# Wangshihu12/Voxel-SLAM

Measured on AMD Instinct MI355X. Metric: local-BA iterations/sec (200k pts, W=10), higher is better.
Workload: dtype f64

## Files before the change

include/voxelba.h:

```cpp
#ifndef VOXELBA_H
#define VOXELBA_H

#include <stddef.h>
#include <stdint.h>

#ifdef __cplusplus
extern "C" {
#endif

#define VBA_CLUSTER_LEN 10
#define VBA_POSE_LEN 12
#define VBA_STATE_LEN 25
#define VBA_IMU_PRE_LEN 304
#define VBA_DIM 15
#define VBA_MAX_WIN 16

enum vba_status {
  VBA_OK = 0,
  VBA_ERR_NO_DEVICE = 1,
  VBA_ERR_BAD_ARG = 2,
  VBA_ERR_UNSUPPORTED_WINDOW = 3,
  VBA_ERR_TOO_FEW_VOXELS = 4,
  VBA_ERR_OPT_STATE = 5,
  VBA_ERR_HIP = 6,
// ... 124 lines not shown

int vba_pgo_optimize(vba_ctx *ctx, int n, double *poses, int m, const double *edges, int n_prior, const double *priors,
                     int n_updates, double relin_threshold, double *stats);

typedef int (*vba_allreduce_fn)(void *user, void *buf_dev, size_t n_doubles, void *stream);
int vba_set_allreduce(vba_ctx *ctx, vba_allreduce_fn fn, void *user);
int vba_rccl_get_unique_id(void *out128);
int vba_rccl_init(vba_ctx *ctx, const void *unique_id128, int rank, int n_ranks);
int vba_set_rccl_comm(vba_ctx *ctx, void *nccl_comm);
int vba_shard_owner(int64_t kx, int64_t ky, int64_t kz, int n_ranks);
int vba_set_shard(vba_ctx *ctx, int rank, int n_ranks);

int vba_timing_enable(vba_ctx *ctx, int on);
int vba_timing_calibration_read(vba_ctx *ctx, size_t n_bytes);
int vba_timing_select(vba_ctx *ctx, const char *name);
int vba_timing_sample_every(vba_ctx *ctx, int n);
int vba_timing_null_span(vba_ctx *ctx);
int vba_timing_reset(vba_ctx *ctx);
int vba_timing_get(vba_ctx *ctx, const char *name, double *total_us, int *count);

int vba_lm_begin(vba_ctx *ctx, const double *poses, int thd_num);
int vba_lm_refresh_eigen(vba_ctx *ctx);
int vba_timing_launch_hessian(vba_ctx *ctx);
int vba_lm_iterate(vba_ctx *ctx, int *accepted, int *stop);
int vba_lm_end(vba_ctx *ctx, double *poses, double *hess, double *resis2);
#define VBA_SOLVE_LIDAR 0
#define VBA_SOLVE_LI 1
#define VBA_SOLVE_DENSE 2
#define VBA_SOLVE_E_PACKED 1
#define VBA_SOLVE_COPY_RAW 2
#define VBA_SOLVE_FROM_RAW 4
#define VBA_SOLVE_GRAVITY 8
#define VBA_SOLVE_DENSE_MASK 16
int vba_debug_solve(vba_ctx *ctx, int kind, int W, int flags, const double *H, const double *g, double u, double v, double *dx, double *q1);

int vba_io_save_pcd(const char *path, int n, const double *xyz);
int vba_io_load_pcd(const char *path, int cap, double *xyz, double *intensity , int *n_out);
int vba_io_save_pose(const char *path, int n, const double *states, const double *v6);
int vba_io_read_lidarstate(const char *path, int cap, double *states, double *v6 , int *n_out);

#define VBA_BTC_ROW_LEN 19

typedef struct vba_btc_config {
  int skip_near_num;
  int candidate_num;
  float rough_dis_threshold;
  float similarity_threshold;
  float icp_threshold;
  float normal_threshold;
  float dis_threshold;
  int occupy_len;
} vba_btc_config;

typedef struct vba_btc_db vba_btc_db;

typedef struct vba_btc_result {
  int loop_id;
  double score;
  double t[3];
  double R[9];
} vba_btc_result;

typedef struct vba_btc_candidate {
  int frame;
  int votes;
  int match_len;
// ... 82 lines not shown
```

voxel-slam_amd/capi.py:

```python
from __future__ import annotations

import ctypes as C
import os
import subprocess

import numpy as np

_PKG = os.path.dirname(os.path.abspath(__file__))
LIB_PATH = os.environ.get("VBA_LIB") or os.path.join(_PKG, "libvoxelba.so")
_dp = C.POINTER(C.c_double)

OK = 0
ERR_NO_DEVICE, ERR_BAD_ARG, ERR_UNSUPPORTED_WINDOW, ERR_TOO_FEW_VOXELS, ERR_OPT_STATE, ERR_HIP, ERR_CAPACITY, ERR_IO, ERR_UNSUPPORTED, ERR_SINGULAR = range(1, 11)

EXPORTS = [
    "vba_default_options", "vba_create", "vba_destroy", "vba_status_string", "vba_last_error", "vba_synchronize",
    "vba_factor_clear", "vba_factor_push_voxels", "vba_factor_size", "vba_factor_acc_evaluate2",
    "vba_factor_evaluate_only_residual", "vba_factor_read_back", "vba_factor_occupied_slots", "vba_factor_occupancy_masks",
    "vba_lidar_ba_damping_iter", "vba_li_ba_damping_iter", "vba_last_lm_trace",
    "vba_imu_preintegrate", "vba_imu_give_evaluate",
    "vba_map_cut_voxel", "vba_map_pvec_update_cut_voxel", "vba_scan_var_init", "vba_scan_down_sampling_voxel", "vba_scan_down_sampling_pvec", "vba_scan_down_sampling_close", "vba_scan_undistort", "vba_odom_lio_state_estimation_kdtree", "vba_odom_kdtree_reset", "vba_odom_kdtree_size", "vba_odom_kdtree_points", "vba_gba_build", "vba_hba_add_edge", "vba_hba_global", "vba_map_cut_voxel_fix", "vba_map_recut", "vba_map_margi", "vba_map_slide", "vba_map_prune", "vba_map_reset",
    "vba_map_num_roots", "vba_map_num_slide_roots", "vba_map_stats", "vba_map_dump_leaves", "vba_map_dump_plane_var", "vba_odom_lio_state_estimation",
    "vba_set_allreduce", "vba_rccl_get_unique_id", "vba_rccl_init", "vba_set_rccl_comm", "vba_shard_owner", "vba_set_shard",
    "vba_timing_enable", "vba_timing_calibration_read", "vba_timing_select", "vba_timing_sample_every", "vba_timing_launch_hessian", "vba_timing_null_span", "vba_timing_reset", "vba_timing_get",
# ... 587 lines not shown

    def factor_occupancy(self) -> float:
        n = C.c_longlong(0)
        self._chk(self.lib.vba_factor_occupied_slots(self.h, C.byref(n)))
        return n.value / max(self.size(), 1)

    def factor_occupancy_masks(self):
        m = np.zeros(self.size(), dtype=np.uint32)
        self._chk(self.lib.vba_factor_occupancy_masks(self.h, m.ctypes.data_as(C.POINTER(C.c_uint))))
        return m

    def last_trace(self):
        rows = np.zeros((64, 5))
        n = self.lib.vba_last_lm_trace(self.h, _p(rows), C.c_int(64))
        return rows[:n].copy()

    def lidar_ba_damping_iter(self, poses, max_iter=3, thd_num=2):
        poses = _c(poses).copy(); n = 6 * self.W
        H = np.empty((n, n)); resis = np.zeros(2); conv = C.c_int(0)
        st = self.lib.vba_lidar_ba_damping_iter(self.h, _p(poses), _p(H), _p(resis), C.c_int(max_iter), C.c_int(thd_num), C.byref(conv))
        if st == ERR_TOO_FEW_VOXELS:
            return dict(poses=poses, hess=H, resis=resis, converge=False, status=-1, trace=self.last_trace())
        self._chk(st)
        return dict(poses=poses, hess=H, resis=resis, converge=bool(conv.value), status=0, trace=self.last_trace())

    def li_ba_damping_iter(self, states, imus, gravity=False, max_iter=3):
        states = _c(states).copy(); imus = _c(imus).copy()
        n = 15 * self.W + (3 if gravity else 0)
        H = np.empty((n, n)); resis = np.zeros(2)
        self._chk(self.lib.vba_li_ba_damping_iter(self.h, _p(states), _p(imus), C.c_int(int(gravity)), C.c_int(max_iter), _p(H), _p(resis)))
        return dict(states=states, imus=imus, hess=H, resis=resis, trace=self.last_trace())

    SOLVE_KINDS = {"lidar": 0, "li": 1, "dense": 2}
    SOLVE_FLAGS = {"e_packed": 1, "copy_raw": 2, "from_raw": 4, "gravity": 8, "dense_mask": 16}

    def debug_solve(self, kind, W, H, g, u, v=2.0, **flags):
        f = 0
        for k, on in flags.items():
            f |= self.SOLVE_FLAGS[k] if on else 0
        H = _c(H); g = _c(g); n = len(g)
        nc = 1 if kind == "dense" else (self.opt.lm_spec if 0 < self.opt.lm_spec < 4 else 4)
        dx = np.zeros((nc, n)); q1 = np.zeros(nc)
        self._chk(self.lib.vba_debug_solve(self.h, C.c_int(self.SOLVE_KINDS[kind]), C.c_int(W), C.c_int(f), _p(H), _p(g),
                                           C.c_double(u), C.c_double(v), _p(dx), _p(q1)))
        return dx, q1

    def lm_begin(self, poses, thd_num=2):
        poses = _c(poses)
        self._chk(self.lib.vba_lm_begin(self.h, _p(poses), C.c_int(thd_num)))

    def lm_iterate(self, sync=True):
        if not sync:
            self._chk(self.lib.vba_lm_iterate(self.h, None, None))
            return None
        acc = C.c_int(0); stop = C.c_int(0)
        self._chk(self.lib.vba_lm_iterate(self.h, C.byref(acc), C.byref(stop)))
        return bool(acc.value), bool(stop.value)

    def lm_refresh_eigen(self):
        self._chk(self.lib.vba_lm_refresh_eigen(self.h))

    def lm_end(self, fetch=True):
        if not fetch:
            self._chk(self.lib.vba_lm_end(self.h, None, None, None))
            return None
        n = 6 * self.W
        poses = np.empty((self.W, 12)); H = np.empty((n, n)); resis = np.zeros(2)
# ... 329 lines not shown
```

voxel-slam_amd/csrc/vba_kernels_factor.hpp:

```cpp
#pragma once
#include <hip/hip_runtime.h>
#include "vba_eig3.hpp"

namespace vba {

struct FactorView {
  double *cl;
  double *fix;
  double *coe;
  double *eigval;
  double *eigvec;
  double *pcr;
  unsigned int *occ;
  int *tiles;
  int vs;
  int W;
};

__host__ __device__ inline int mask_bucket(unsigned int m, int nb) {
  constexpr int C[11][11] = {{1, 0, 0, 0, 0, 0, 0, 0, 0, 0, 0}, {1, 1, 0, 0, 0, 0, 0, 0, 0, 0, 0}, {1, 2, 1, 0, 0, 0, 0, 0, 0, 0, 0}, {1, 3, 3, 1, 0, 0, 0, 0, 0, 0, 0},
                             {1, 4, 6, 4, 1, 0, 0, 0, 0, 0, 0}, {1, 5, 10, 10, 5, 1, 0, 0, 0, 0, 0}, {1, 6, 15, 20, 15, 6, 1, 0, 0, 0, 0},
                             {1, 7, 21, 35, 35, 21, 7, 1, 0, 0, 0}, {1, 8, 28, 56, 70, 56, 28, 8, 1, 0, 0}, {1, 9, 36, 84, 126, 126, 84, 36, 9, 1, 0},
                             {1, 10, 45, 120, 210, 252, 210, 120, 45, 10, 1}};
  int p = 0;
// ... 163 lines not shown
__device__ __forceinline__ double wave_sum(double x) {
  for (int m = 32; m >= 1; m >>= 1) x += __shfl_xor(x, m, 64);
  return x;
}

__device__ __forceinline__ double dpp_mov_f64(double x, double old, const int ctrl, const int row_mask) {
  const long long xi = __double_as_longlong(x), oi = __double_as_longlong(old);
  int lo = (int)xi, hi = (int)(xi >> 32);
  const int olo = (int)oi, ohi = (int)(oi >> 32);
  switch (ctrl) {
    case 0xB1: lo = __builtin_amdgcn_update_dpp(olo, lo, 0xB1, 0xF, 0xF, false); hi = __builtin_amdgcn_update_dpp(ohi, hi, 0xB1, 0xF, 0xF, false); break;
    case 0x4E: lo = __builtin_amdgcn_update_dpp(olo, lo, 0x4E, 0xF, 0xF, false); hi = __builtin_amdgcn_update_dpp(ohi, hi, 0x4E, 0xF, 0xF, false); break;
    case 0x141: lo = __builtin_amdgcn_update_dpp(olo, lo, 0x141, 0xF, 0xF, false); hi = __builtin_amdgcn_update_dpp(ohi, hi, 0x141, 0xF, 0xF, false); break;
    case 0x140: lo = __builtin_amdgcn_update_dpp(olo, lo, 0x140, 0xF, 0xF, false); hi = __builtin_amdgcn_update_dpp(ohi, hi, 0x140, 0xF, 0xF, false); break;
    case 0x142: lo = __builtin_amdgcn_update_dpp(olo, lo, 0x142, 0xA, 0xF, false); hi = __builtin_amdgcn_update_dpp(ohi, hi, 0x142, 0xA, 0xF, false); break;
    default: lo = __builtin_amdgcn_update_dpp(olo, lo, 0x143, 0xC, 0xF, false); hi = __builtin_amdgcn_update_dpp(ohi, hi, 0x143, 0xC, 0xF, false); break;
  }
  (void)row_mask;
  return __longlong_as_double(((long long)hi << 32) | (unsigned int)lo);
}
__device__ __forceinline__ double group8_sum(double x) {
  x += dpp_mov_f64(x, x, 0xB1, 0xF);
  x += dpp_mov_f64(x, x, 0x4E, 0xF);
  x += dpp_mov_f64(x, x, 0x141, 0xF);
  return x;
}
__device__ __forceinline__ double wave_sum_to_lane63(double x) {
  x += dpp_mov_f64(x, x, 0xB1, 0xF);
  x += dpp_mov_f64(x, x, 0x4E, 0xF);
  x += dpp_mov_f64(x, x, 0x141, 0xF);
  x += dpp_mov_f64(x, x, 0x140, 0xF);
  x += dpp_mov_f64(x, 0.0, 0x142, 0xA);
  x += dpp_mov_f64(x, 0.0, 0x143, 0xC);
  return x;
}

struct LmDev;
template <int W>
struct LmInit {
  double x[12 * W];
  LmDev *dst;
  int on, dbg;
};
template <int W>
__device__ __forceinline__ void lm_init_store(const LmInit<W> &a, int tid, int nt);

template <int W, int TV>
struct ResCfg {
  static constexpr int NT = ((TV * W + 63) / 64) * 64;
  static constexpr int NF = NT / TV;
  static constexpr int KPT = (10 + NF - 1) / NF;
  static_assert(TV <= 64 && (TV & (TV - 1)) == 0 && NT % TV == 0, "the voxel threads are the first TV lanes of wave 0");
  static_assert(W * 12 <= NT, "one thread per pose scalar");
};

template <int W, int TV, bool STAMPS>
__global__ __launch_bounds__((ResCfg<W, TV>::NT)) void k_residual_s(FactorView f, const double *__restrict__ poses, int head, int end,
                                                                  double *__restrict__ partial, const int *__restrict__ gate,
                                                                  long long *__restrict__ stamps, LmInit<W> init) {
  using C = ResCfg<W, TV>;
  __shared__ double T[10][W][TV];
  __shared__ double S[10][TV];
  __shared__ double sp[W * 12];
  const int gate_v = gate ? *gate : 1;
  const int tid = threadIdx.x, vl = tid % TV, fi = tid / TV;
  const int v = head + blockIdx.x * TV + vl;
// ... 576 lines not shown
```

voxel-slam_amd/csrc/vba_kernels_li.hpp:

```cpp
#pragma once
#include <hip/hip_runtime.h>
#include "vba_hostmath.hpp"
#include "vba_li_order.hpp"

namespace vba {

constexpr int LI_MAX_W = 16;
constexpr int LI_MAX_N = 15 * LI_MAX_W + 3;

struct LiDev {
  int W, n, nb, gravity, gauge, F;
  double imu_coef;
  double ex[LI_MAX_W * 12];
  double ext[LI_MAX_W * 12];
  double tstamp[LI_MAX_W];
  double rimu[2];
  double ext_spec[LM_SPEC][LI_MAX_W * 12];
  double ginc_spec[LM_SPEC][4];
  double binc_spec[LM_SPEC][LI_MAX_W * 6];
};

__device__ __forceinline__ void li_state(const double *pose12, const double *ex12, double t, vbh::State &s) {
  s.t = t;
#pragma unroll
// ... 168 lines not shown
  using LC = LdltCfg<NP>;
  extern __shared__ __attribute__((aligned(16))) double lds[];
  const int sb = blockIdx.x;
  constexpr size_t LSCR = (size_t)LC::LTOT > (size_t)NMAX * (NMAX + 1) / 2 ? (size_t)LC::LTOT : (size_t)NMAX * (NMAX + 1) / 2;
  double *Lst = GL ? lscratch + (size_t)sb * LSCR : lds, *Tp = GL ? lds : Lst + LC::LTOT, *P = Tp + NP * LC::LS;
  double *hd = P + NP * 8, *gs = hd + NMAX, *dsh = gs + NMAX, *xs = dsh + NMAX, *dxs = xs + NP, *red8 = dxs + NMAX;
  int *ord = (int *)(red8 + 32);
  const int tid = threadIdx.x;
  const long long t_begin = clock64();
  constexpr int NLB = (2 * W - 1) * 225, NLOW = NLB + 45 * W + 9, QH = (NLOW + NT - 1) / NT, NL = 36 * W * W, QL = (NL + NT - 1) / NT;
  const int nlow = NLB + (grav ? 45 * W + 9 : 0);
  double hv[QH], lv[QL];
#pragma unroll
  for (int q = 0; q < QH; q++) {
    const int e = tid + NT * q, ec = e < nlow ? e : 0;
    int idx;
    if (ec < NLB) { const int blk = ec / 225, a = (blk + 1) >> 1, b = a - (blk & 1); idx = li_hb_pair(a, b) + (ec - 225 * blk); }
    else idx = li_hb_ne1(W) + 45 * W + (ec - NLB);
    hv[q] = himu[idx];
  }
  if (!copy_raw) {
#pragma unroll
    for (int q = 0; q < QL; q++) {
      const int e = tid + NT * q, ec = e < NL ? e : NL - 1;
      const int row = ec / (6 * W), col = ec - row * (6 * W);
      lv[q] = tl_fetch<W>(red, row, col);
    }
  }
  double gimu_v = 0.0, glid_v = 0.0;
  if (tid < n) {
    gimu_v = gimu[tid];
    if (!copy_raw && tid < 15 * W) { const int a = tid / 15, lr = tid - 15 * a; glid_v = (lr < 6) ? red[C2::GB + 6 * a + lr] : 0.0; }
  }
  const int stop = s->stop, calc = s->is_calc_hess, iter0 = s->iter, dbg = sb == 0 ? s->pad : 0, use_spec = s->use_spec;
  const double u0 = s->u, v0 = s->v, rimu0 = li->rimu[0], rlid0 = copy_raw ? 0.0 : red[C2::RB];
  if (stop || use_spec) return;
  double u = u0;
  { double vb = v0; for (int k = 0; k < sb; k++) { u = u * vb; vb = 2 * vb; } }
  if ((dbg & 16) && tid == 0) s->stamps[0] = t_begin;
  const double *__restrict__ src = (copy_raw && !calc) ? raw : red;
  if (copy_raw) {
    if (calc && sb == 0)
      for (int t = tid; t < C2::NOUT2; t += NT) raw[t] = src[t];
#pragma unroll
    for (int q = 0; q < QL; q++) {
      const int e = tid + NT * q, ec = e < NL ? e : NL - 1;
      const int row = ec / (6 * W), col = ec - row * (6 * W);
      lv[q] = tl_fetch<W>(src, row, col);
    }
    if (tid < 15 * W) { const int a = tid / 15, lr = tid - 15 * a; glid_v = (lr < 6) ? src[C2::GB + 6 * a + lr] : 0.0; }
  }
  if (tid == 0 && calc && sb == 0) {
    const double rl = copy_raw ? src[C2::RB] : rlid0, r = coef * 0.5 * rimu0 + rl;
    s->r1 = r; if (iter0 == 0) s->resis_first = r;
    if ((dbg & 32) && iter0 < 3) { s->stamps[58 + 2 * iter0] = __double_as_longlong(rimu0); s->stamps[59 + 2 * iter0] = __double_as_longlong(rl); }
  }
  double *stage = Lst;
  for (int e = tid; e < n * (n + 1) / 2; e += NT) stage[e] = 0.0;
  __syncthreads();
#pragma unroll
  for (int q = 0; q < QH; q++) {
    const int e = tid + NT * q;
    if (e < nlow) {
      int R, Cc;
      if (e < NLB) { const int blk = e / 225, rc = e - 225 * blk, a = (blk + 1) >> 1, b = a - (blk & 1); R = 15 * a + rc / 15; Cc = 15 * b + rc % 15; }
      else if (e < NLB + 45 * W) { const int q2 = e - NLB, k = q2 / (15 * W); R = 15 * W + k; Cc = q2 - k * 15 * W; }
      else { const int q2 = e - NLB - 45 * W; R = 15 * W + q2 / 3; Cc = 15 * W + q2 % 3; }
// ... 9 lines not shown
    if (e < NL && col <= row) {
      const int R = 15 * (row / 6) + row % 6, Cc = 15 * (col / 6) + col % 6;
      stage[R * (R + 1) / 2 + Cc] += lv[q];
    }
  }
  __syncthreads();
  if ((dbg & 16) && tid == 0) s->stamps[51] = clock64();
  if (tid < n) {
    double h = 1.0, g = 0.0;
    if (tid >= gauge) {
      h = stage[tid * (tid + 1) / 2 + tid];
      g = coef * gimu_v + glid_v;
    }
    hd[tid] = h; gs[tid] = g; dsh[tid] = fabs(h + u * h);
  }
  __syncthreads();
  if ((dbg & 16) && tid == 0) s->stamps[52] = clock64();
  if (tid < n) ord[tid] = li_ord(tid, W);
  __syncthreads();
  auto elem = [&](int i, int j) -> double {
    const int jc = j < n ? j : n - 1, ic = i < n ? i : n - 1;
    const int pj = ord[jc], pi = ord[ic];
    const int rr = pi > pj ? pi : pj, cc = pi > pj ? pj : pi;
    double a = stage[rr * (rr + 1) / 2 + cc];
    a = (rr < gauge || cc < gauge) ? ((rr == cc) ? 1.0 : 0.0) : a;
    a = (i == j) ? a + u * a : a;
    a = (i == n) ? -gs[pj] : a;
    a = (i > n || i < j) ? 0.0 : a;
    return (j >= n) ? ((i == j) ? 1.0 : 0.0) : a;
  };
  long long *stamps = ((dbg & 16) != 0) ? s->stamps : nullptr;
  if (stamps && tid == 0) stamps[1] = clock64();
  auto live = [&](int kb) -> unsigned { return li_live(kb, W, n, NP); };
  if constexpr (DENSE_MASK) ldlt_mfma<NP, NT>(Lst, Tp, P, n, elem, stamps, LdltDense());
  else ldlt_mfma<NP, NT>(Lst, Tp, P, n, elem, stamps, live);
  if (stamps && tid == 0) stamps[3] = clock64();
  if (tid < n) xs[tid] = Lst[LC::lat(n, tid)];
  __syncthreads();
  const double x = ldlt_backsub<NP>(Lst, xs, n);
  if (stamps && tid == 0) stamps[4] = clock64();
  if (tid < n) dxs[ord[tid]] = x;
  __syncthreads();
  double *gl = red8 + 16;
  if (grav && tid < 3) {
    if (sb == 0) { const double gn = li->ext[9 + tid] + dxs[n - 3 + tid]; gl[tid] = gn; }
    else li->ginc_spec[sb][tid] = dxs[n - 3 + tid];
  }
  __syncthreads();
  if (tid < W) {
    double E[9];
    so3_exp_dev(dxs + 15 * tid, E);
    const double *R = s->x + 12 * tid;
    double *Rt = (sb == 0 ? s->xt : s->xt_spec[sb]) + 12 * tid;
    double *et = (sb == 0 ? li->ext : li->ext_spec[sb]) + 12 * tid;
    for (int r = 0; r < 3; r++)
      for (int c = 0; c < 3; c++) Rt[3 * r + c] = R[3 * r] * E[c] + R[3 * r + 1] * E[3 + c] + R[3 * r + 2] * E[6 + c];
    for (int k = 0; k < 3; k++) Rt[9 + k] = R[9 + k] + dxs[15 * tid + 3 + k];
    for (int k = 0; k < 9; k++) et[k] = li->ex[12 * tid + k] + dxs[15 * tid + 6 + k];
    if (grav && sb == 0) for (int k = 0; k < 3; k++) et[9 + k] = gl[k];
  }
  if (tid >= 64 && tid < 64 + li->F) {
    const int f = tid - 64;
    if (sb == 0) {
      double *m = imu + 304 * (size_t)f;
      for (int k = 0; k < 3; k++) {
        m[73 + k] = m[67 + k]; m[76 + k] = m[70 + k];
        m[67 + k] += dxs[15 * f + 9 + k]; m[70 + k] += dxs[15 * f + 12 + k];
      }
    } else {
// ... 123 lines not shown
```

voxel-slam_amd/csrc/vba_kernels_lm.hpp:

```cpp
#pragma once
#include <hip/hip_runtime.h>
#include "vba_ldlt.hpp"

namespace vba {

constexpr int LM_SPEC = 4;

struct LmDev {
  double x[VBA_MAX_WIN_DEV * 12];
  double xt[VBA_MAX_WIN_DEV * 12];
  double u, v, r1, r2, q1, resis_first;
  int is_calc_hess, stop, iter, n_trace, all_accepted, last_accepted, max_trace, run_hess, run_res, pad;
  double trace[5 * 64];
  long long stamps[64];
  int spec_n, spec_i, use_spec, pad2;
  double q1_spec[LM_SPEC];
  double xt_spec[LM_SPEC][VBA_MAX_WIN_DEV * 12];
};

template <int W>
__device__ __forceinline__ void lm_init_store(const LmInit<W> &a, int tid, int nt) {
  constexpr int NW = sizeof(LmDev) / 8, XT = offsetof(LmDev, xt) / 8, U = offsetof(LmDev, u) / 8, V = offsetof(LmDev, v) / 8,
                I = offsetof(LmDev, is_calc_hess) / 8;
  static_assert(sizeof(LmDev) % 8 == 0 && offsetof(LmDev, x) == 0 && offsetof(LmDev, u) == 2 * offsetof(LmDev, xt) && 12 * W <= XT, "x and xt lead the image");
// ... 87 lines not shown
      }
  };
  if constexpr (!COPY_RAW) { load_diag(red); load_bulk(red); }
  const double r_v = COPY_RAW ? 0.0 : red[C2::RB];
  double xr[12];
  if (wv == 3 && lane < W)
#pragma unroll
    for (int k = 0; k < 12; k++) xr[k] = s->x[12 * lane + k];
  const long long t_begin = clock64();
  if (stop || use_spec) return;
  double u = u0;
  { double vb = v0; for (int k = 0; k < sb; k++) { u = u * vb; vb = 2 * vb; } }
  if constexpr (COPY_RAW) {
    const double *__restrict__ src = calc ? red : raw;
    if (calc && sb == 0)
      for (int t = tid; t < C2::NOUT2; t += NT) raw[t] = src[t];
    load_diag(src); load_bulk(src);
  }
  double hk[NH], dk[NH];
  int rk[NH];
#pragma unroll
  for (int h = 0; h < NH; h++) {
    const int k = lane + 64 * h;
    hk[h] = k < 6 ? 1.0 : dgt[h] + dge[h];
    dk[h] = fabs(hk[h] + u * hk[h]);
    rk[h] = 0;
  }
#pragma unroll
  for (int j = 0; j < n; j++) {
    const double o = readlane_f64(dk[j >> 6], j & 63);
#pragma unroll
    for (int h = 0; h < NH; h++) rk[h] += (o > dk[h] || (o == dk[h] && j < lane + 64 * h)) ? 1 : 0;
  }
  int prow[T16], pcol[T16];
#pragma unroll
  for (int t = 0; t < T16; t++) {
    const int r = 16 * t + ru, c = 16 * t + cu;
    prow[t] = __shfl(rk[(16 * t) >> 6], (r < n ? r : n - 1) & 63);
    pcol[t] = __shfl(rk[(16 * t) >> 6], (c < n ? c : n - 1) & 63);
  }
  {
    int uu = 0;
#pragma unroll
    for (int ta = 0; ta < T16; ta++)
#pragma unroll
      for (int tb = ta; tb < T16; tb++, uu++) {
        const int row = 16 * ta + ru, col = 16 * tb + cu;
        if (row <= col && col < n) {
          double a = eon[uu] ? tv[uu] + ev[uu] : tv[uu];
          a = (row < 6) ? ((row == col) ? 1.0 : 0.0) : a;
          a = (row == col) ? a + u * a : a;
          const int pr = prow[ta], pc = pcol[tb], hi = pr > pc ? pr : pc, lo = pr > pc ? pc : pr;
          img[hi * (hi + 1) / 2 + lo] = a;
        }
      }
  }
  if (wv == 0)
#pragma unroll
    for (int h = 0; h < NH; h++) {
      const int k = lane + 64 * h;
      if (k < n) {
        const double g = k < 6 ? 0.0 : gv[h];
        hd[k] = hk[h]; gs[k] = g; ord[rk[h]] = k;
        img[n * (n + 1) / 2 + rk[h]] = -g;
      }
    }
#pragma unroll
  for (int i = n; i < NP; i++)
    if (tid <= i && (i > n || tid >= n)) img[i * (i + 1) / 2 + tid] = (tid == i) ? 1.0 : 0.0;
  const int iter0 = s->iter, dbg = s->pad;
  if (tid == 0 && calc && sb == 0) { const double r = COPY_RAW ? red[C2::RB] : r_v; s->r1 = r; if (iter0 == 0) s->resis_first = r; }
  long long *stamps = ((dbg & 16) && tid == 0 && sb == 0) ? s->stamps : nullptr;
  if (stamps) stamps[0] = t_begin;
  __syncthreads();
  auto elem = [&](int i, int j) -> double {
    return img[i >= j ? i * (i + 1) / 2 + j : ZERO];
  };
  if (stamps) stamps[1] = clock64();
  ldlt_mfma<NP, NT>(Lst, Tp, P, n, elem, ((dbg & 16) && sb == 0) ? s->stamps : nullptr);
  if (stamps) stamps[3] = clock64();
  if (tid < n) xs[tid] = Lst[LC::lat(n, tid)];
  __syncthreads();
  const double x = ldlt_backsub<NP>(Lst, xs, n);
  if (stamps) stamps[4] = clock64();
  if (tid < n) dxs[ord[tid]] = x;
  __syncthreads();
  if (wv == 3) {
    if (lane < W) {
      double E[9];
      so3_exp_dev(dxs + 6 * lane, E);
      const double *R = xr;
      double *Rt = (sb == 0 ? s->xt : s->xt_spec[sb]) + 12 * lane;
#pragma unroll
      for (int r = 0; r < 3; r++)
#pragma unroll
        for (int c = 0; c < 3; c++) Rt[3 * r + c] = R[3 * r] * E[c] + R[3 * r + 1] * E[3 + c] + R[3 * r + 2] * E[6 + c];
#pragma unroll
      for (int k = 0; k < 3; k++) Rt[9 + k] = R[9 + k] + dxs[6 * lane + 3 + k];
    }
    if (lane == 63) red8[3] = 0.0;
  } else {
    double q = tid < n ? dxs[tid] * (u * hd[tid] * dxs[tid] - gs[tid]) : 0.0;
    q = wave_sum_to_lane63(q);
    if (lane == 63) red8[wv] = q;
  }
  __syncthreads();
  if (dx_out && tid < n) dx_out[sb * n + tid] = dxs[tid];
  if (tid == 0) {
    const double q1 = 0.5 * (red8[0] + red8[1] + red8[2] + red8[3]);
    s->q1_spec[sb] = q1;
    if (sb == 0) { s->q1 = q1; s->spec_n = gridDim.x; s->spec_i = 0; }
  }
  if (stamps) stamps[5] = clock64();
}
// ... 93 lines not shown
```

voxel-slam_amd/csrc/vba_ldlt.hpp:

```cpp
#pragma once
#include <hip/hip_runtime.h>

namespace vba {

typedef double v4f64_l __attribute__((ext_vector_type(4)));

__device__ __forceinline__ double readlane_f64(double v, int lane) {
  int lo = __double2loint(v), hi = __double2hiint(v);
  lo = __builtin_amdgcn_readlane(lo, lane);
  hi = __builtin_amdgcn_readlane(hi, lane);
  return __hiloint2double(hi, lo);
}

template <int NP>
struct LdltCfg {
  static constexpr int NTL = NP / 16, NTILES = NTL * (NTL + 1) / 2, NBLK = NP / 8, LS = 9;
  static constexpr int LTOT = LS * 4 * NBLK * (NBLK + 1);
  __host__ __device__ static constexpr int lst_off(int kb) { return LS * 8 * (kb * NBLK - kb * (kb - 1) / 2); }
  static constexpr int DOUBLES = LTOT + NP * LS + NP * 8;
  __device__ static __forceinline__ int lat(int j, int i) { return lst_off(i >> 3) + (j - (i & ~7)) * LS + (i & 7); }
};

struct LdltDense { __device__ __forceinline__ unsigned operator()(int) const { return ~0u; } };
template <int NP, int NT, typename F, typename LV = LdltDense>
__device__ __forceinline__ void ldlt_mfma(double *__restrict__ Lst, double *__restrict__ Tp, double *__restrict__ P, int rhs_row, F elem, long long *stamps = nullptr, LV live = LV()) {
  using C = LdltCfg<NP>;
  constexpr int NW = NT / 64, TPW = (C::NTILES + NW - 1) / NW, LS = C::LS;
  const int tid = threadIdx.x, l = tid & 63, w = tid >> 6, lr = l >> 4, lc = l & 15;
  int tti[TPW], ttj[TPW];
  v4f64_l acc[TPW];
#pragma unroll
  for (int u = 0; u < TPW; u++) {
    const int t = w + NW * u;
    int tj = C::NTL - 1, rem = t;
    while (tj > 0 && rem >= C::NTL - tj) { rem -= C::NTL - tj; tj--; }
    tti[u] = tj + rem; ttj[u] = tj;
    if (t < C::NTILES) {
#pragma unroll
      for (int r = 0; r < 4; r++) acc[u][r] = elem(16 * tti[u] + lr + 4 * r, 16 * ttj[u] + lc);
      if (ttj[u] == 0 && lc < 8)
#pragma unroll
        for (int r = 0; r < 4; r++) P[(16 * tti[u] + lr + 4 * r) * 8 + lc] = acc[u][r];
    }
  }
  if (stamps && tid == 0) stamps[2] = clock64();
  for (int kb = 0; kb < C::NBLK; kb++) {
    const int k0 = 8 * kb;
    double *Lk = Lst + C::lst_off(kb);
    __syncthreads();
    if (stamps && tid == 0 && kb < 20) stamps[8 + 2 * kb] = clock64();
    if ((tid | 63) >= k0 && (tid & ~63) < NP) {
      const bool rowlane = tid < NP && tid >= k0;
      const int i = rowlane ? tid : k0, ib = i - k0;
      double Dr[8], x[8];
      {
        const double *dr = P + (k0 + (l & 7)) * 8;
        const double2 d0 = *reinterpret_cast<const double2 *>(dr), d1 = *reinterpret_cast<const double2 *>(dr + 2),
                      d2 = *reinterpret_cast<const double2 *>(dr + 4), d3 = *reinterpret_cast<const double2 *>(dr + 6);
        Dr[0] = d0.x; Dr[1] = d0.y; Dr[2] = d1.x; Dr[3] = d1.y; Dr[4] = d2.x; Dr[5] = d2.y; Dr[6] = d3.x; Dr[7] = d3.y;
        const double2 x0 = *reinterpret_cast<const double2 *>(P + i * 8), x1 = *reinterpret_cast<const double2 *>(P + i * 8 + 2),
                      x2 = *reinterpret_cast<const double2 *>(P + i * 8 + 4), x3 = *reinterpret_cast<const double2 *>(P + i * 8 + 6);
        x[0] = x0.x; x[1] = x0.y; x[2] = x1.x; x[3] = x1.y; x[4] = x2.x; x[5] = x2.y; x[6] = x3.x; x[7] = x3.y;
      }
      const bool is_rhs = rowlane && (i == rhs_row);
#pragma unroll
      for (int c = 0; c < 8; c++) {
        const double d = readlane_f64(Dr[c], c);
        const bool ok = fabs(d) > 0.0;
        const double y0 = __builtin_amdgcn_rcp(d);
        const double e = fma(-d, y0, 1.0);
        const double y1 = fma(e, y0, y0), e2 = e * e;
        const double inv = fma(e2, y1, y1);
        const double dinv = ok ? inv : 0.0;
        double lv = ok ? x[c] * dinv : x[c];
        if (is_rhs) lv = (fabs(d) > 2.2250738585072014e-308) ? x[c] * dinv : 0.0;
        lv = (ib > c) ? lv : 0.0;
        const double tmc = (ok && ib > c) ? x[c] : 0.0;
        if (rowlane) { Lk[ib * LS + c] = lv; Tp[i * LS + c] = -tmc; }
        const double lrc = Dr[c] * dinv;
#pragma unroll
        for (int c2 = c + 1; c2 < 8; c2++) {
          const double Lc2 = readlane_f64(lrc, c2);
          x[c2] = fma(-tmc, Lc2, x[c2]);
          Dr[c2] = fma(-Dr[c], Lc2, Dr[c2]);
        }
      }
    }
    __syncthreads();
    if (stamps && tid == 0 && kb < 20) stamps[9 + 2 * kb] = clock64();
    const int kn = k0 + 8;
    if (kn >= NP) break;
    const int tjn = kn >> 4, cb0 = kn & 15;
    const unsigned lm = (unsigned)__builtin_amdgcn_readfirstlane((int)live(kb));
    double la0[TPW], la1[TPW], tb0[TPW], tb1[TPW];
    bool actv[TPW];
#pragma unroll
    for (int u = 0; u < TPW; u++) {
      const bool act = (w + NW * u < C::NTILES) && (ttj[u] >= tjn) && ((lm >> tti[u]) & 1u) && ((lm >> ttj[u]) & 1u);
      actv[u] = act;
      const double *la = Lk + (act ? (16 * tti[u] + lc - k0) : 0) * LS + lr, *tb = Tp + (act ? (16 * ttj[u] + lc) : k0) * LS + lr;
      la0[u] = la[0]; la1[u] = la[4]; tb0[u] = tb[0]; tb1[u] = tb[4];
    }
#pragma unroll
    for (int u = 0; u < TPW; u++)
      if (actv[u]) acc[u] = __builtin_amdgcn_mfma_f64_16x16x4f64(la0[u], tb0[u], acc[u], 0, 0, 0);
#pragma unroll
    for (int u = 0; u < TPW; u++) {
      if (actv[u]) acc[u] = __builtin_amdgcn_mfma_f64_16x16x4f64(la1[u], tb1[u], acc[u], 0, 0, 0);
      if ((w + NW * u < C::NTILES) && ttj[u] == tjn && lc >= cb0 && lc < cb0 + 8)
#pragma unroll
        for (int r = 0; r < 4; r++) P[(16 * tti[u] + lr + 4 * r) * 8 + (lc - cb0)] = acc[u][r];
    }
  }
  __syncthreads();
}

template <int NP>
__device__ __forceinline__ double ldlt_backsub(const double *__restrict__ Lst, double *__restrict__ xs, int n) {
  using C = LdltCfg<NP>;
  const int tid = threadIdx.x, wv = tid >> 6;
  const int nblk = (n + 63) >> 6;
  double x = (tid < n) ? xs[tid] : 0.0;
  for (int b = nblk - 1; b >= 0; b--) {
    const int hiR = (64 * b + 63 < n - 1) ? 64 * b + 63 : n - 1;
// ... 35 lines not shown
```

voxel-slam_amd/csrc/voxelba.hip:

```cpp
#include "../../include/voxelba.h"

#define VBA_MAX_WIN_DEV VBA_MAX_WIN
#include "vba_kernels_factor.hpp"
#include "vba_kernels_h3.hpp"
#include "vba_kernels_map.hpp"
#include "vba_kernels_lm.hpp"
#include "vba_kernels_li.hpp"
#include "vba_kernels_scan.hpp"
#include "vba_kernels_gba.hpp"
#include "vba_kernels_big.hpp"
#include "vba_kernels_pgo.hpp"
#include "vba_kernels_kd.hpp"
#include "vba_kernels_init.hpp"
#include "vba_kernels_btc.hpp"
#include "vba_btcgen.hpp"
#include "vba_io.hpp"
#include <cstddef>
#include "vba_hostmath.hpp"

#include <hip/hip_runtime.h>
#include <rccl/rccl.h>
#include <dlfcn.h>
#include <cstdio>
#include <cstdlib>
// ... 883 lines not shown
  if (st) return st;
  if (!want) {
    hipLaunchKernelGGL(k_lm_update, dim3(1), dim3(64), 0, c->stream, c->d_lm, c->d_k4part, c->lm.k4_nb, W);
    c->lm.pending_update = false;
    c->lm.active = false;
    return VBA_OK;
  }
  double *h_hess = nullptr;
  if (hess) {
    st = ensure_pin(c, 65536 + (size_t)n * n + 1024);
    if (st) return st;
    h_hess = c->h_pin + 32768;
  }
  const double *src = c->collective() ? c->d_raw : c->d_out;
  const int upd = c->lm.pending_update ? 1 : 0;
  switch (W) {
#define VBA_FIN_CASE(WW) case WW: hipLaunchKernelGGL(k_lm_finish<WW>, dim3(hess ? 17 : 1), dim3(256), 0, c->stream, c->d_lm, c->d_k4part, upd ? c->lm.k4_nb : 0, upd, c->h_lm, src, h_hess); break;
    VBA_FIN_CASE(2) VBA_FIN_CASE(3) VBA_FIN_CASE(4) VBA_FIN_CASE(5) VBA_FIN_CASE(6) VBA_FIN_CASE(7) VBA_FIN_CASE(8) VBA_FIN_CASE(9) VBA_FIN_CASE(10)
    VBA_FIN_CASE(11) VBA_FIN_CASE(12) VBA_FIN_CASE(13) VBA_FIN_CASE(14) VBA_FIN_CASE(15) VBA_FIN_CASE(16)
#undef VBA_FIN_CASE
    default: return VBA_ERR_UNSUPPORTED_WINDOW;
  }
  c->lm.pending_update = false;
  HIPCHK(c, hipGetLastError());
  HIPCHK(c, hipStreamSynchronize(c->stream));
  const LmDev *h = c->h_lm;
  if (poses) std::memcpy(poses, h->x, (size_t)W * 12 * sizeof(double));
  if (hess) std::memcpy(hess, c->h_pin + 32768, (size_t)n * n * sizeof(double));
  if (resis2) { resis2[0] = h->resis_first; resis2[1] = h->r2; }
  c->trace.assign(h->trace, h->trace + 5 * h->n_trace);
  if (h->pad & 16) {
    fprintf(stderr, "[k_lm_solve_m cycles] prologue %lld | tile load %lld | factorisation %lld | backsub %lld | epilogue %lld | panels:", h->stamps[1] - h->stamps[0],
            h->stamps[2] - h->stamps[1], h->stamps[3] - h->stamps[2], h->stamps[4] - h->stamps[3], h->stamps[5] - h->stamps[4]);
    for (int kb = 0; kb < 8; kb++) fprintf(stderr, " %lld+%lld", h->stamps[9 + 2 * kb] - h->stamps[8 + 2 * kb], kb < 7 ? h->stamps[10 + 2 * kb] - h->stamps[9 + 2 * kb] : 0LL);
    fprintf(stderr, "\n");
  }
  c->lm.active = false;
  return VBA_OK;
}

int vba_lidar_ba_damping_iter(vba_ctx *c, double *poses, double *hess, double *resis2, int max_iter, int thd_num, int *is_converge) {
  int st = vba_lm_begin(c, poses, thd_num);
  if (st) return st;
  for (int i = 0; i < max_iter; i++) {
    st = vba_lm_iterate(c, nullptr, nullptr);
    if (st) { c->lm.active = false; return st; }
  }
  st = vba_lm_end(c, poses, hess, resis2);
  if (is_converge) *is_converge = c->h_lm->all_accepted;
  return st;
}

int vba_last_lm_trace(vba_ctx *c, double *rows, int max_rows) {
  int n = (int)(c->trace.size() / 5);
  if (n > max_rows) n = max_rows;
  if (rows) std::memcpy(rows, c->trace.data(), (size_t)n * 5 * sizeof(double));
  return n;
}

extern "C++" {
template <int W>
struct LiSolveCfg {
  static constexpr int NMAX = 15 * W + 3, NP = ((NMAX + 1 + 15) / 16) * 16;
  static constexpr bool GL = W > 10;
  static constexpr size_t l_doubles = (size_t)LdltCfg<NP>::LTOT > (size_t)NMAX * (NMAX + 1) / 2 ? (size_t)LdltCfg<NP>::LTOT : (size_t)NMAX * (NMAX + 1) / 2;
  static constexpr size_t lds = ((GL ? (size_t)LdltCfg<NP>::DOUBLES - LdltCfg<NP>::LTOT : (size_t)LdltCfg<NP>::DOUBLES) + 4 * NMAX + NP + 32) * 8 + (size_t)NMAX * 4 + 64;
  static_assert(GL || l_doubles == (size_t)LdltCfg<NP>::LTOT, "the staged triangle must fit the region of L");
};
// ... 163 lines not shown
  hipLaunchKernelGGL(k_pack_segments, dim3(64, segs.n), dim3(256), 0, c->stream, segs, c->d_lipack);
  HIPCHK(c, hipGetLastError());
  HIPCHK(c, hipMemcpyAsync(c->h_pin, c->d_lipack, o_end * sizeof(double), hipMemcpyDeviceToHost, c->stream));
  HIPCHK(c, hipStreamSynchronize(c->stream));
  std::memcpy(c->h_lm, c->h_pin + o_lm, sizeof(LmDev));
  std::memcpy(&h, c->h_pin + o_li, sizeof(LiDev));
  std::memcpy(fimg.data(), c->h_pin + o_img, fimg.size() * sizeof(double));
  const double *himu_h = c->h_pin + o_hb;
  c->lm.active = false;
  const LmDev *hl = c->h_lm;
  for (int i = 0; i < W; i++) {
    double *sx = states + 25 * i;
    for (int k = 0; k < 12; k++) sx[1 + k] = hl->x[12 * i + k];
    for (int k = 0; k < 12; k++) sx[13 + k] = h.ex[12 * i + k];
  }
  if (hl->use_spec)
    for (int f = 0; f < F; f++) std::memcpy(fimg.data() + 304 * (size_t)f + 67, fimg.data() + 304 * (size_t)f + 73, 6 * sizeof(double));
  for (int f = 0; f < F; f++) std::memcpy(imus + 304 * (size_t)f + 67, fimg.data() + 304 * (size_t)f + 67, 12 * sizeof(double));
  if (hess) {
    const double *lid = c->h_pin + o_lid;
    for (int r = 0; r < n; r++)
      for (int k = 0; k < n; k++) hess[(size_t)r * n + k] = c->opt.imu_coef * li_hb_get(himu_h, W, n, r, k);
    for (int i = 0; i < W; i++)
      for (int j = 0; j < W; j++)
        for (int r = 0; r < 6; r++)
          for (int k = 0; k < 6; k++) hess[(size_t)(i * DIM + r) * n + j * DIM + k] += lid[(size_t)(i * 6 + r) * n6 + j * 6 + k];
  }
  if (gravity && resis2) { resis2[0] = hl->resis_first; resis2[1] = hl->r2; }
  c->trace.assign(hl->trace, hl->trace + 5 * hl->n_trace);
  if (want_times && (hl->pad & 16)) {
    fprintf(stderr, "[k_li_solve prologue] stage imu %lld | stage lidar %lld | diag+g %lld | rank %lld\n", hl->stamps[50] - hl->stamps[0], hl->stamps[51] - hl->stamps[50], hl->stamps[52] - hl->stamps[51], hl->stamps[1] - hl->stamps[52]);
    fprintf(stderr, "[k_li_solve cycles] prologue %lld | tile load %lld | factorisation %lld | backsub %lld | epilogue %lld | panels:", hl->stamps[1] - hl->stamps[0],
            hl->stamps[2] - hl->stamps[1], hl->stamps[3] - hl->stamps[2], hl->stamps[4] - hl->stamps[3], hl->stamps[5] - hl->stamps[4]);
    for (int kb = 0; kb < 20; kb++) fprintf(stderr, " %lld+%lld", hl->stamps[9 + 2 * kb] - hl->stamps[8 + 2 * kb], kb < 19 ? hl->stamps[10 + 2 * kb] - hl->stamps[9 + 2 * kb] : 0LL);
    fprintf(stderr, "\n");
  }
  if (want_times && (hl->pad & 64)) fprintf(stderr, "[k_li_imu cycles] factor algebra (one lane per factor) %lld | cov^-1 joc %lld | contractions %lld\n", hl->stamps[41] - hl->stamps[40], hl->stamps[42] - hl->stamps[41], hl->stamps[43] - hl->stamps[42]);
  if (want_times && (hl->pad & 32)) { double v[6]; std::memcpy(v, &hl->stamps[58], sizeof(v)); fprintf(stderr, "[li r1 parts] rank %d: rimu %.10g lidar %.10g | %.10g %.10g | %.10g %.10g\n", c->rank, v[0], v[1], v[2], v[3], v[4], v[5]); }
  if (want_times) fprintf(stderr, "[li_ba_device] upload %.1f us | enqueue %.1f | gpu drained at %.1f | total %.1f\n", t_up, t_enq - t_up, t_gpu, since(t_0));
  return VBA_OK;
}

int vba_li_ba_damping_iter(vba_ctx *c, double *states, double *imus, int gravity, int max_iter, double *hess, double *resis2) {
  if (!li_device_supported(c->opt.win_size)) return VBA_ERR_UNSUPPORTED_WINDOW;
  return li_ba_device(c, states, imus, gravity, max_iter, hess, resis2);
}

static int kd_reserve(vba_ctx *c, size_t pts) {
  if (pts <= c->kd_cap) return VBA_OK;
  size_t cap = c->kd_cap ? c->kd_cap : 65536;
  while (cap < pts) cap *= 2;
  for (int i = 0; i < 2; i++) {
    double *nw = nullptr;
    HIPCHK(c, hipMalloc((void **)&nw, cap * 3 * sizeof(double)));
    if (c->d_kdtree[i]) {
      if (i == c->kd_cur && c->kd_n > 0) HIPCHK(c, hipMemcpyAsync(nw, c->d_kdtree[i], (size_t)c->kd_n * 3 * sizeof(double), hipMemcpyDeviceToDevice, c->stream));
      HIPCHK(c, hipStreamSynchronize(c->stream));
      hipFree(c->d_kdtree[i]);
    }
    c->d_kdtree[i] = nw;
  }
  c->kd_cap = cap;
  return VBA_OK;
}
int vba_odom_kdtree_reset(vba_ctx *c) { c->kd_n = 0; return VBA_OK; }
int vba_odom_kdtree_size(vba_ctx *c) { return c->kd_n; }
int vba_odom_kdtree_points(vba_ctx *c, double *out) {
  if (!out && c->kd_n > 0) return VBA_ERR_BAD_ARG;
// ... 2430 lines not shown
    }
  }
  const int ncand = kind == VBA_SOLVE_DENSE ? 1 : c->lm_spec;
  {
    double ub = u, vb = v;
    if (!std::isfinite(u) || !std::isfinite(v)) return VBA_ERR_BAD_ARG;
    for (int k = 1; k < ncand; k++) { ub = ub * vb; vb = 2 * vb; if (!std::isfinite(ub) || !std::isfinite(vb)) return VBA_ERR_BAD_ARG; }
  }
  HIPCHK(c, hipSetDevice(c->device));
  std::vector<LmDev> hv(1);
  DbgBufs B(c->stream);
  if (kind == VBA_SOLVE_DENSE) {
    BigStore S;
    S.b.W = W; S.NP = (n + 7) / 8 * 8; S.ld = (S.NP + 63) / 64 * 64;
    HIPCHK(c, B.alloc(&S.b.H, (size_t)n * n)); HIPCHK(c, B.alloc(&S.b.g, (size_t)n));
    HIPCHK(c, B.alloc(&S.d_Ab, (size_t)(S.NP + 1) * S.ld)); HIPCHK(c, B.alloc(&S.d_Tb, (size_t)(S.NP + 1) * 8));
    HIPCHK(c, B.alloc(&S.d_ord, (size_t)n)); HIPCHK(c, B.alloc(&S.d_vec, (size_t)3 * n));
    HIPCHK(c, hipMemcpyAsync(S.b.H, H, (size_t)n * n * sizeof(double), hipMemcpyHostToDevice, c->stream));
    HIPCHK(c, hipMemcpyAsync(S.b.g, g, (size_t)n * sizeof(double), hipMemcpyHostToDevice, c->stream));
    std::vector<double> hd(n), jt(g, g + n);
    std::vector<int> ord(n);
    for (int r = 0; r < n; r++) hd[r] = H[(size_t)r * n + r];
    for (int r = 0; r < 6; r++) { hd[r] = 1.0; jt[r] = 0.0; }
    big_pivot_order(hd.data(), u, n, ord.data());
    const int st = big_solve(S, c->stream, ord.data(), u, dx, c->err);
    if (st) return st;
    q1[0] = big_q1(dx, hd.data(), jt.data(), u, n);
    return VBA_OK;
  }
  LmDev *h = hv.data();
  std::memset(h, 0, sizeof(LmDev));
  for (int f = 0; f < W; f++) { h->x[12 * f] = h->x[12 * f + 4] = h->x[12 * f + 8] = 1.0; }
  h->u = u; h->v = v;
  double *d_dx = nullptr;
  HIPCHK(c, B.alloc(&d_dx, (size_t)ncand * n));
  int st = VBA_ERR_BAD_ARG;
  switch (W) {
#define VBA_DS_CASE(WW) case WW: st = kind == VBA_SOLVE_LIDAR ? dbg_lidar<WW>(c, B, H, g, flags, *h, d_dx) : dbg_li<WW>(c, B, H, g, flags, *h, d_dx); break;
    VBA_DS_CASE(2) VBA_DS_CASE(3) VBA_DS_CASE(4) VBA_DS_CASE(5) VBA_DS_CASE(6) VBA_DS_CASE(7) VBA_DS_CASE(8) VBA_DS_CASE(9) VBA_DS_CASE(10)
    VBA_DS_CASE(11) VBA_DS_CASE(12) VBA_DS_CASE(13) VBA_DS_CASE(14) VBA_DS_CASE(15) VBA_DS_CASE(16)
#undef VBA_DS_CASE
  }
  if (st) return st;
  HIPCHK(c, hipMemcpyAsync(dx, d_dx, (size_t)ncand * n * sizeof(double), hipMemcpyDeviceToHost, c->stream));
  HIPCHK(c, hipStreamSynchronize(c->stream));
  for (int b = 0; b < ncand; b++) q1[b] = h->q1_spec[b];
  return VBA_OK;
}

}

#include "vba_kernels_kf.hpp"

struct vba_kf_store {
  vba_ctx *ctx = nullptr;
  double *d_pnt = nullptr; float *d_var = nullptr; size_t cap = 0;
  std::vector<int> off{0};
  struct Meta { double x0[12]; int id; double jour; int exist; };
  std::vector<Meta> kf;
  size_t mcap = 0;
  double *d_src = nullptr, *d_merge = nullptr, *d_mdiag = nullptr, *h_diag = nullptr;
  int *d_cnt = nullptr; char *d_ws = nullptr; size_t ws_bytes = 0;
  int tcap = 0; char *h_tab = nullptr, *d_tab = nullptr; int *h_n = nullptr;
  hipEvent_t ev = nullptr;
  int allocs = 0; int64_t bytes = 0;
  int hist = 0; std::vector<float> hist_pos;
// ... 803 lines not shown
```

Baseline: 22460.

## Stop LDLT factorisation after the last panel that holds live pivoted columns

The lidar LM solve kernel now computes, through a wave-wide DPP max reduction, the highest pivot rank among the non-fixed columns and runs only that many 8-column panels of the MFMA LDLT factorisation instead of all NP padded panels. The unfactored trailing panels of L are zeroed so the unchanged back-substitution still works. The LDLT routine takes a new column-count argument, and a debug flag (pad bit 128 / ALL_PANELS) restores full factorisation. The aim is to avoid factoring padded columns; the cost is an extra rank reduction and the risk of a wrong solution if the rank bound misses a live column.

```diff
diff --git a/include/voxelba.h b/include/voxelba.h
--- a/include/voxelba.h
+++ b/include/voxelba.h
@@ -180,6 +180,7 @@
 #define VBA_SOLVE_FROM_RAW 4
 #define VBA_SOLVE_GRAVITY 8
 #define VBA_SOLVE_DENSE_MASK 16
+#define VBA_SOLVE_ALL_PANELS 32
 int vba_debug_solve(vba_ctx *ctx, int kind, int W, int flags, const double *H, const double *g, double u, double v, double *dx, double *q1);
 
 int vba_io_save_pcd(const char *path, int n, const double *xyz);
diff --git a/voxel-slam_amd/capi.py b/voxel-slam_amd/capi.py
--- a/voxel-slam_amd/capi.py
+++ b/voxel-slam_amd/capi.py
@@ -643,7 +643,7 @@
         return dict(states=states, imus=imus, hess=H, resis=resis, trace=self.last_trace())
 
     SOLVE_KINDS = {"lidar": 0, "li": 1, "dense": 2}
-    SOLVE_FLAGS = {"e_packed": 1, "copy_raw": 2, "from_raw": 4, "gravity": 8, "dense_mask": 16}
+    SOLVE_FLAGS = {"e_packed": 1, "copy_raw": 2, "from_raw": 4, "gravity": 8, "dense_mask": 16, "all_panels": 32}
 
     def debug_solve(self, kind, W, H, g, u, v=2.0, **flags):
         f = 0
diff --git a/voxel-slam_amd/csrc/vba_kernels_factor.hpp b/voxel-slam_amd/csrc/vba_kernels_factor.hpp
--- a/voxel-slam_amd/csrc/vba_kernels_factor.hpp
+++ b/voxel-slam_amd/csrc/vba_kernels_factor.hpp
@@ -219,6 +219,16 @@
   x += dpp_mov_f64(x, x, 0x140, 0xF);
   x += dpp_mov_f64(x, 0.0, 0x142, 0xA);
   x += dpp_mov_f64(x, 0.0, 0x143, 0xC);
+  return x;
+}
+__device__ __forceinline__ int wave_max_to_lane63(int x) {
+  auto mx = [](int a, int b) { return a > b ? a : b; };
+  x = mx(x, __builtin_amdgcn_update_dpp(x, x, 0xB1, 0xF, 0xF, false));
+  x = mx(x, __builtin_amdgcn_update_dpp(x, x, 0x4E, 0xF, 0xF, false));
+  x = mx(x, __builtin_amdgcn_update_dpp(x, x, 0x141, 0xF, 0xF, false));
+  x = mx(x, __builtin_amdgcn_update_dpp(x, x, 0x140, 0xF, 0xF, false));
+  x = mx(x, __builtin_amdgcn_update_dpp(0, x, 0x142, 0xA, 0xF, false));
+  x = mx(x, __builtin_amdgcn_update_dpp(0, x, 0x143, 0xC, 0xF, false));
   return x;
 }
 
diff --git a/voxel-slam_amd/csrc/vba_kernels_li.hpp b/voxel-slam_amd/csrc/vba_kernels_li.hpp
--- a/voxel-slam_amd/csrc/vba_kernels_li.hpp
+++ b/voxel-slam_amd/csrc/vba_kernels_li.hpp
@@ -224,7 +224,7 @@
     gimu_v = gimu[tid];
     if (!copy_raw && tid < 15 * W) { const int a = tid / 15, lr = tid - 15 * a; glid_v = (lr < 6) ? red[C2::GB + 6 * a + lr] : 0.0; }
   }
-  const int stop = s->stop, calc = s->is_calc_hess, iter0 = s->iter, dbg = sb == 0 ? s->pad : 0, use_spec = s->use_spec;
+  const int stop = s->stop, calc = s->is_calc_hess, iter0 = s->iter, dmask = s->pad, dbg = sb == 0 ? dmask : 0, use_spec = s->use_spec;
   const double u0 = s->u, v0 = s->v, rimu0 = li->rimu[0], rlid0 = copy_raw ? 0.0 : red[C2::RB];
   if (stop || use_spec) return;
   double u = u0;
@@ -300,9 +300,10 @@
   long long *stamps = ((dbg & 16) != 0) ? s->stamps : nullptr;
   if (stamps && tid == 0) stamps[1] = clock64();
   auto live = [&](int kb) -> unsigned { return li_live(kb, W, n, NP); };
-  if constexpr (DENSE_MASK) ldlt_mfma<NP, NT>(Lst, Tp, P, n, elem, stamps, LdltDense());
-  else ldlt_mfma<NP, NT>(Lst, Tp, P, n, elem, stamps, live);
-  if (stamps && tid == 0) stamps[3] = clock64();
+  const int ncols = (dmask & 128) ? NP : n;
+  if constexpr (DENSE_MASK) ldlt_mfma<NP, NT>(Lst, Tp, P, n, elem, stamps, LdltDense(), ncols);
+  else ldlt_mfma<NP, NT>(Lst, Tp, P, n, elem, stamps, live, ncols);
+  if (stamps && tid == 0) { stamps[3] = clock64(); stamps[6] = (ncols + 7) / 8 < LC::NBLK ? (ncols + 7) / 8 : LC::NBLK; }
   if (tid < n) xs[tid] = Lst[LC::lat(n, tid)];
   __syncthreads();
   const double x = ldlt_backsub<NP>(Lst, xs, n);
diff --git a/voxel-slam_amd/csrc/vba_kernels_lm.hpp b/voxel-slam_amd/csrc/vba_kernels_lm.hpp
--- a/voxel-slam_amd/csrc/vba_kernels_lm.hpp
+++ b/voxel-slam_amd/csrc/vba_kernels_lm.hpp
@@ -143,6 +143,14 @@
 #pragma unroll
     for (int h = 0; h < NH; h++) rk[h] += (o > dk[h] || (o == dk[h] && j < lane + 64 * h)) ? 1 : 0;
   }
+  int rmax = 0;
+#pragma unroll
+  for (int h = 0; h < NH; h++) {
+    const int k = lane + 64 * h;
+    rmax = (k >= 6 && k < n && rk[h] > rmax) ? rk[h] : rmax;
+  }
+  rmax = wave_max_to_lane63(rmax);
+  const int npan = __builtin_amdgcn_readlane(rmax, 63) / 8 + 1;
   int prow[T16], pcol[T16];
 #pragma unroll
   for (int t = 0; t < T16; t++) {
@@ -188,9 +196,12 @@
     return img[i >= j ? i * (i + 1) / 2 + j : ZERO];
   };
   if (stamps) stamps[1] = clock64();
-  ldlt_mfma<NP, NT>(Lst, Tp, P, n, elem, ((dbg & 16) && sb == 0) ? s->stamps : nullptr);
-  if (stamps) stamps[3] = clock64();
-  if (tid < n) xs[tid] = Lst[LC::lat(n, tid)];
+  const int ncols = (dbg & 128) ? NP : 8 * npan, nsol = ncols < n ? ncols : n;
+  ldlt_mfma<NP, NT>(Lst, Tp, P, n, elem, ((dbg & 16) && sb == 0) ? s->stamps : nullptr, LdltDense(), ncols);
+  if (stamps) { stamps[3] = clock64(); stamps[6] = (ncols + 7) / 8 < LC::NBLK ? (ncols + 7) / 8 : LC::NBLK; }
+  if (tid < n) xs[tid] = tid < nsol ? Lst[LC::lat(n, tid)] : 0.0;
+  for (int kb = (nsol + 7) >> 3; 8 * kb < n; kb++)
+    for (int e = tid; e < (n - 8 * kb) * LC::LS; e += NT) Lst[LC::lst_off(kb) + e] = 0.0;
   __syncthreads();
   const double x = ldlt_backsub<NP>(Lst, xs, n);
   if (stamps) stamps[4] = clock64();
diff --git a/voxel-slam_amd/csrc/vba_ldlt.hpp b/voxel-slam_amd/csrc/vba_ldlt.hpp
--- a/voxel-slam_amd/csrc/vba_ldlt.hpp
+++ b/voxel-slam_amd/csrc/vba_ldlt.hpp
@@ -23,8 +23,9 @@
 
 struct LdltDense { __device__ __forceinline__ unsigned operator()(int) const { return ~0u; } };
 template <int NP, int NT, typename F, typename LV = LdltDense>
-__device__ __forceinline__ void ldlt_mfma(double *__restrict__ Lst, double *__restrict__ Tp, double *__restrict__ P, int rhs_row, F elem, long long *stamps = nullptr, LV live = LV()) {
+__device__ __forceinline__ void ldlt_mfma(double *__restrict__ Lst, double *__restrict__ Tp, double *__restrict__ P, int rhs_row, F elem, long long *stamps = nullptr, LV live = LV(), int ncols = NP) {
   using C = LdltCfg<NP>;
+  const int nc = __builtin_amdgcn_readfirstlane(ncols < NP ? ncols : NP);
   constexpr int NW = NT / 64, TPW = (C::NTILES + NW - 1) / NW, LS = C::LS;
   const int tid = threadIdx.x, l = tid & 63, w = tid >> 6, lr = l >> 4, lc = l & 15;
   int tti[TPW], ttj[TPW];
@@ -44,7 +45,7 @@
     }
   }
   if (stamps && tid == 0) stamps[2] = clock64();
-  for (int kb = 0; kb < C::NBLK; kb++) {
+  for (int kb = 0; 8 * kb < nc; kb++) {
     const int k0 = 8 * kb;
     double *Lk = Lst + C::lst_off(kb);
     __syncthreads();
@@ -89,7 +90,7 @@
     __syncthreads();
     if (stamps && tid == 0 && kb < 20) stamps[9 + 2 * kb] = clock64();
     const int kn = k0 + 8;
-    if (kn >= NP) break;
+    if (kn >= nc) break;
     const int tjn = kn >> 4, cb0 = kn & 15;
     const unsigned lm = (unsigned)__builtin_amdgcn_readfirstlane((int)live(kb));
     double la0[TPW], la1[TPW], tb0[TPW], tb1[TPW];
diff --git a/voxel-slam_amd/csrc/voxelba.hip b/voxel-slam_amd/csrc/voxelba.hip
--- a/voxel-slam_amd/csrc/voxelba.hip
+++ b/voxel-slam_amd/csrc/voxelba.hip
@@ -939,8 +939,9 @@
   if (h->pad & 16) {
     fprintf(stderr, "[k_lm_solve_m cycles] prologue %lld | tile load %lld | factorisation %lld | backsub %lld | epilogue %lld | panels:", h->stamps[1] - h->stamps[0],
             h->stamps[2] - h->stamps[1], h->stamps[3] - h->stamps[2], h->stamps[4] - h->stamps[3], h->stamps[5] - h->stamps[4]);
-    for (int kb = 0; kb < 8; kb++) fprintf(stderr, " %lld+%lld", h->stamps[9 + 2 * kb] - h->stamps[8 + 2 * kb], kb < 7 ? h->stamps[10 + 2 * kb] - h->stamps[9 + 2 * kb] : 0LL);
-    fprintf(stderr, "\n");
+    const int npr = (int)h->stamps[6];
+    for (int kb = 0; kb < npr && kb < 8; kb++) fprintf(stderr, " %lld+%lld", h->stamps[9 + 2 * kb] - h->stamps[8 + 2 * kb], kb < npr - 1 ? h->stamps[10 + 2 * kb] - h->stamps[9 + 2 * kb] : 0LL);
+    fprintf(stderr, " | %d panels run\n", npr);
   }
   c->lm.active = false;
   return VBA_OK;
@@ -1170,8 +1171,9 @@
     fprintf(stderr, "[k_li_solve prologue] stage imu %lld | stage lidar %lld | diag+g %lld | rank %lld\n", hl->stamps[50] - hl->stamps[0], hl->stamps[51] - hl->stamps[50], hl->stamps[52] - hl->stamps[51], hl->stamps[1] - hl->stamps[52]);
     fprintf(stderr, "[k_li_solve cycles] prologue %lld | tile load %lld | factorisation %lld | backsub %lld | epilogue %lld | panels:", hl->stamps[1] - hl->stamps[0],
             hl->stamps[2] - hl->stamps[1], hl->stamps[3] - hl->stamps[2], hl->stamps[4] - hl->stamps[3], hl->stamps[5] - hl->stamps[4]);
-    for (int kb = 0; kb < 20; kb++) fprintf(stderr, " %lld+%lld", hl->stamps[9 + 2 * kb] - hl->stamps[8 + 2 * kb], kb < 19 ? hl->stamps[10 + 2 * kb] - hl->stamps[9 + 2 * kb] : 0LL);
-    fprintf(stderr, "\n");
+    const int npr = (int)hl->stamps[6];
+    for (int kb = 0; kb < npr && kb < 20; kb++) fprintf(stderr, " %lld+%lld", hl->stamps[9 + 2 * kb] - hl->stamps[8 + 2 * kb], kb < npr - 1 ? hl->stamps[10 + 2 * kb] - hl->stamps[9 + 2 * kb] : 0LL);
+    fprintf(stderr, " | %d panels run\n", npr);
   }
   if (want_times && (hl->pad & 64)) fprintf(stderr, "[k_li_imu cycles] factor algebra (one lane per factor) %lld | cov^-1 joc %lld | contractions %lld\n", hl->stamps[41] - hl->stamps[40], hl->stamps[42] - hl->stamps[41], hl->stamps[43] - hl->stamps[42]);
   if (want_times && (hl->pad & 32)) { double v[6]; std::memcpy(v, &hl->stamps[58], sizeof(v)); fprintf(stderr, "[li r1 parts] rank %d: rimu %.10g lidar %.10g | %.10g %.10g | %.10g %.10g\n", c->rank, v[0], v[1], v[2], v[3], v[4], v[5]); }
@@ -3668,6 +3670,7 @@
   std::memset(h, 0, sizeof(LmDev));
   for (int f = 0; f < W; f++) { h->x[12 * f] = h->x[12 * f + 4] = h->x[12 * f + 8] = 1.0; }
   h->u = u; h->v = v;
+  if (flags & VBA_SOLVE_ALL_PANELS) h->pad = 128;
   double *d_dx = nullptr;
   HIPCHK(c, B.alloc(&d_dx, (size_t)ncand * n));
   int st = VBA_ERR_BAD_ARG;
```

Measured after the change: 22970 (median of 6 runs). 1.02x the previous value.
